# ProteusMRIgHIFU/BabelBrain

Measured on AMD Instinct MI355X. Metric: Mvoxel-steps/sec, 512^3 skull FDTD per device (achieved HBM GB/s in roofline), higher is better.
Workload: dtype f32

## Files before the change

babelbrain_amd/csrc/bfd_api.hip:

```cpp
#include "bfd_internal.h"

#include <math.h>
#include <stdio.h>
#include <string.h>

#include <algorithm>
#include <array>
#include <thread>
#include <hipcub/hipcub.hpp>

static thread_local std::string g_err;
void bfd_set_error(const std::string &s) { g_err = s; }

namespace {

struct HostTables {
    std::vector<float> t;
    float c1, k2;
    double cmax;
};

void fit_sls(double rho, double c, double alpha, double q, double omega, bool exact, double &MR, double &tau)
{
    if (c <= 0.0) { MR = 0.0; tau = 0.0; return; }
// ... 469 lines not shown
        BFD_FAIL(-2, "bfd_create: h, dt, freq must be > 0 and 0 < reflectionLimit < 1");
    int ndev = 0;
    if (hipGetDeviceCount(&ndev) != hipSuccess || ndev <= 0)
        BFD_FAIL(-3, "bfd_create: no HIP device available (this engine has no CPU fallback)");
    if (cfg->device < 0 || cfg->device >= ndev) BFD_FAIL(-3, "bfd_create: device ordinal out of range");
    BFD_HIP(hipSetDevice(cfg->device));

    bfd_sim *s = new bfd_sim();
    s->cfg = *cfg;
    s->step = 0; s->devBytes = 0; s->haveMaterials = s->haveMap = false; s->tilesReady = false;
    s->nSrcVox = 0; s->srcLin = s->srcRow = nullptr; s->srcW[0] = s->srcW[1] = s->srcW[2] = nullptr; s->pulseT = nullptr;
    s->nSources = s->lengthSource = 0;
    s->pulseHost = nullptr; s->tileSteps = s->nTiles = 0;
    s->srcK = 0; s->srcWeights = s->srcSignals = nullptr;
    for (int b = 0; b < 2; b++) { s->tileDev[b] = s->tilePinned[b] = nullptr; s->tileLoaded[b] = s->tilePacked[b] = -1; s->evTile[b] = nullptr; s->evTileUsed[b] = false; for (int q = 0; q < 2; q++) { s->evRead[b][q] = nullptr; s->evReadUsed[b][q] = false; } }
    s->sensEnt = nullptr; s->sensEntValid = false; s->sensIsBox = false; memset(s->sensBox, 0, sizeof s->sensBox);
    s->actBase = nullptr; s->actBytes = 0; s->actReady = false;
    s->nSensors = 0; s->sensLin = nullptr; s->sensOut = nullptr; s->dftAcc = nullptr; s->dftPk = nullptr; s->dftBin = 0;
    s->acc = s->pk = nullptr; s->timing = s->perKernel = false;
    s->pairEnv = true; s->pendingAcc = s->pairDone = false; s->pairedLaunches = 0;
    if (const char *ev = getenv("BFD_PAIR_ACC")) s->pairEnv = atoi(ev) != 0;
    s->advEnv = true; s->midStep = false; s->tiles.advVz = false;
    if (const char *ev = getenv("BFD_ADV_VZ")) s->advEnv = atoi(ev) != 0;
    s->tables = nullptr; s->profiles = nullptr; s->cmax = 0;
    memset(s->algBytes, 0, sizeof s->algBytes); s->tiles.ktimer = nullptr;
    if (hipStreamCreateWithFlags(&s->stream, hipStreamNonBlocking) != hipSuccess) { delete s; BFD_FAIL(-10, "hipStreamCreate failed"); }
    s->ownStream = true;
    if (hipEventCreate(&s->evBegin) != hipSuccess) { hipStreamDestroy(s->stream); delete s; BFD_FAIL(-10, "hipEventCreate failed"); }
    if (hipEventCreate(&s->evEnd) != hipSuccess) { hipEventDestroy(s->evBegin); hipStreamDestroy(s->stream); delete s; BFD_FAIL(-10, "hipEventCreate failed"); }

    bfd_dev &d = s->d;
    memset(&d, 0, sizeof d);
    d.N1 = cfg->N1; d.N2 = cfg->N2; d.N3 = cfg->N3; d.k0 = cfg->k0; d.nk = cfg->nk;
    d.ND = cfg->NDelta; d.P = P; d.plane = cfg->N1 * cfg->N2;
    s->nloc = (size_t)d.plane * d.nk;
    s->nalloc = (size_t)d.plane * (d.nk + 4);
    bfd_placement_cache_evict_other_sizes(cfg->device, s->nalloc * sizeof(float));

    int rc = 0;
    float **fp[15] = {&d.Vx, &d.Vy, &d.Vz, &d.Sxx, &d.Syy, &d.Szz, &d.Sxy, &d.Sxz, &d.Syz,
                      &d.Rxx, &d.Ryy, &d.Rzz, &d.Rxy, &d.Rxz, &d.Ryz};
    for (int a = 0; a < 15 && !rc; a++) {
        rc = dev_alloc(s, &s->stateBase[a], s->nalloc);
        if (!rc) *fp[a] = s->stateBase[a] + 2 * (size_t)d.plane;
    }
    if (!rc) rc = dev_alloc(s, &s->matBase, s->nalloc);
// ... 626 lines not shown
    const bool pairAcc = pair_engine(s, quiet_runs_wanted(s), T.nFluid);
    for (size_t r = 0; r < all.size(); r++) {
        const int4 &run = all[r];
        const int bx = run.x % tx, by = run.x / tx, kb = run.y & 0xFFFF, ke = run.y >> 16, f = run.z;
        const int xa = bx * 64, xb = std::min(xa + 64, N1), ya = by * 8, yb = std::min(ya + 8, N2);
        const double cells = (double)(xb - xa) * (yb - ya) * (ke - kb);
        const double inner = overlap(xa, xb, ND, N1 - ND) * overlap(ya, yb, ND, N2 - ND) * overlap(k0g + kb, k0g + ke, ND, N3 - ND);
        const bool fusedRun = r >= (size_t)(T.nFluid + T.nSolid);
        if (fusedRun) {
            const double fc = 64.0 * bfd_fused_rows() * (ke - kb);
            const double b = 32.0 + ((f & 2) ? 8.0 : 0.0) + ((f & 4) ? 0.0 : 2.0);
            B[0][BFD_K_FUSED] += b * fc; B[1][BFD_K_FUSED] += b * fc + 8.0 * fc;
        } else if (r < (size_t)T.nFluid) {
            const bool lossy = f & 2, uni = f & 4, single = (f & 16) != 0;
            double bs = 12.0 + 8.0 + (lossy ? 8.0 : 0.0) + (uni ? 0.0 : 2.0);
            if (!single) bs += 8.0 + (lossy ? 8.0 : 0.0);
            const double bv = 4.0 + 24.0 + (uni ? 0.0 : 2.0);
            for (int a = 0; a < 2; a++) { B[a][BFD_K_STRESS_FLUID] += bs * cells; B[a][BFD_K_VELOCITY_FLUID] += bv * cells; }
            if (pairAcc) B[1][BFD_K_STRESS_FLUID] += 4.0 * inner; else B[1][BFD_K_VELOCITY_FLUID] += 8.0 * inner;
            if (f & BFD_RUN_ADV_VZ) {
                const double advCells = (double)(xb - xa) * (yb - ya) * std::max(0, ke - kb - 3);
                for (int a = 0; a < 2; a++) { B[a][BFD_K_STRESS_FLUID] += 4.0 * advCells; B[a][BFD_K_VELOCITY_FLUID] -= 8.0 * advCells; }
            }
        } else if (s->cfg.kernelVariant == 2) {
            for (int a = 0; a < 2; a++) { B[a][BFD_K_STRESS_SOLID] += 110.0 * cells; B[a][BFD_K_VELOCITY_SOLID] += 50.0 * cells + (a ? 8.0 * inner : 0.0); }
        } else {
            for (int a = 0; a < 2; a++) B[a][BFD_K_VELOCITY_SOLID] += (a ? 8.0 * inner : 0.0);
        }
    }
    if (T.nSolid && s->cfg.kernelVariant != 2) {
        const double nF0 = (double)cnt[0], nF1 = (double)cnt[1], nS = (double)cnt[2] + (double)cnt[3], nE = (double)cnt[4], nR = (double)cnt[5];
        const double all = nF0 + nF1 + nS + nR;
        const double bs = 15.0 * all + 8.0 * nF0 + 16.0 * nF1 + 48.0 * nS + 48.0 * nR;
        const double bv = 31.0 * all + 8.0 * (nS + nR) + 4.0 * nE;
        const double bsf = 14.0 * all + 8.0 * nF0 + 16.0 * nF1 + 16.0 * nS + 8.0 * nR;
        for (int a = 0; a < 2; a++) { if (s->d.cssRow) B[a][BFD_K_STRESS_FLUID] += bsf; else B[a][BFD_K_STRESS_SOLID] += bs; B[a][BFD_K_VELOCITY_SOLID] += bv; }
    }
    if (s->tiles.nShear) {
        DevTemp<unsigned long long> dc; unsigned long long hc[2] = {0, 0};
        BFD_HIP(dc.alloc(2));
        hipMemsetAsync(dc, 0, sizeof hc, s->stream);
        hipLaunchKernelGGL(count_active_edges, dim3(grid_for(s->tiles.nShear)), dim3(256), 0, s->stream, s->tiles.shearCoef, s->tiles.shearCodes, s->tiles.nShear, dc.p);
        hipMemcpyAsync(hc, dc, sizeof hc, hipMemcpyDeviceToHost, s->stream);
        const hipError_t e = hipStreamSynchronize(s->stream);
        if (e != hipSuccess) BFD_FAIL(-10, std::string("shear edge count: ") + hipGetErrorString(e));
        s->tiles.nShearExplicit = (long)hc[1];
// ... 21 lines not shown
    dev_release(s, &s->tiles.cssRow); dev_release(s, &s->tiles.css); s->tiles.cssCap = 0; s->tiles.cssHosted = false;
    dev_release(s, &s->tiles.runsAll); s->tiles.nAll = s->tiles.nAllB = 0;
    dev_release(s, &s->tiles.runs); dev_release(s, &s->tiles.xmap); dev_release(s, &s->tiles.shearCells); dev_release(s, &s->tiles.shearCoef); dev_release(s, &s->tiles.shearR);
    dev_release(s, &s->tiles.shearCodes); dev_release(s, &s->tiles.shearTab);
    const TileGrid G = choose_tile_grid(s);
    std::vector<int> flags(G.n, 1), mats(G.n, 0);
    if (s->cfg.kernelVariant != 2) { const int rc = fetch_tile_classes(s, G.n, flags, mats); if (rc) return rc; }
    bfd_tiles &T = s->tiles;
    T.nMat = s->cfg.nMat;
    T.nFluid = T.nFluidB = T.nSolid = T.nSolidB = T.nSolidBP = T.nSolidIP = T.nFused = T.nLossless = T.nLossy = T.nSolidSub = T.nUni = T.nPml = T.nLean = T.nFusedSub = 0;
    s->d.tilesX = G.tx; s->d.tilesY = G.ty;
    if (s->cfg.kernelVariant != 2) for (int id = 0; id < G.n; id++) if (!(flags[id] & 1)) flags[id] |= 16;
    std::vector<int4> lists[5];
    std::vector<int4> listsAll[2];
    std::vector<char> taken((size_t)G.n, 0);
    form_fused_runs(s, G, flags, mats, taken, lists[4]);
    form_two_kernel_runs(s, G, flags, mats, taken, lists, listsAll);
    T.nFluidB = (int)lists[0].size(); T.nFluid = T.nFluidB + (int)lists[1].size();
    T.nSolidB = (int)lists[2].size(); T.nSolid = T.nSolidB + (int)lists[3].size();
    T.nFused = (int)lists[4].size();
    T.advVz = false;
    if (adv_vz_engine(s, T.nSolid))
        for (int a = 0; a < 2; a++)
            for (int4 &run : lists[a])
                if (!(run.z & (1 | 8)) && (run.y >> 16) - (run.y & 0xFFFF) >= 4) { run.z |= BFD_RUN_ADV_VZ; T.advVz = true; }
    std::vector<int4> all;
    for (int a = 0; a < 5; a++) all.insert(all.end(), lists[a].begin(), lists[a].end());
    int rc = dev_alloc(s, &s->tiles.runs, all.size(), false);
    if (rc) return rc;
    BFD_HIP(hipMemcpy(s->tiles.runs, all.data(), all.size() * sizeof(int4), hipMemcpyHostToDevice));
    rc = build_balance_maps(s, all);
    if (rc) return rc;
    s->tiles.nShearExplicit = 0;
    s->tiles.nShear = s->tiles.shearLowEnd = s->tiles.shearHighBeg = 0;
    if (T.nSolid && s->cfg.kernelVariant != 2) {
        int count = 0; bool compact = false; std::vector<unsigned> hostCells;
        rc = build_shear_list(s, G, &count, &compact, hostCells);
        if (!rc && compact) rc = setup_compact_state(s, G, count, listsAll);
        if (!rc && carryCompact) rc = carry_compact_in(s, count, oldCells, oldN, oldComp);
        if (!rc && compact && s->step > 0 && !carryCompact) {
            float *comp[10] = {s->d.cSxx, s->d.cSyy, s->d.cSxy, s->d.cSxz, s->d.cSyz, s->d.cRxx, s->d.cRyy, s->d.cRxy, s->d.cRxz, s->d.cRyz};
            for (int a = 0; a < 10; a++) BFD_HIP(hipMemsetAsync(comp[a], 0, (size_t)count * sizeof(float), s->stream));
            BFD_HIP(hipStreamSynchronize(s->stream));
        }
        if (rc) return rc;
        s->tiles.shearLowEnd = std::lower_bound(hostCells.begin(), hostCells.end(), (unsigned)G.lowPlanes * (unsigned)s->d.plane) - hostCells.begin();
        s->tiles.shearHighBeg = std::lower_bound(hostCells.begin(), hostCells.end(), (unsigned)G.hiStart * (unsigned)s->d.plane) - hostCells.begin();
    } else if (carryCompact) {
// ... 480 lines not shown
```

babelbrain_amd/csrc/bfd_internal.h:

```cpp
#pragma once
#include <hip/hip_runtime.h>
#include <stdint.h>
#include <algorithm>
#include <future>
#include <string>
#include <vector>
#include "../../include/babelfdtd.h"

#define BFD_REFLECTOR_BIT 0x8000u
#define BFD_MAT_MASK 0x7FFFu
#define BFD_CLS_FLUID 1u
#define BFD_CLS_NOMEM 2u
#define BFD_CLS_EXY 4u
#define BFD_CLS_EXZ 8u
#define BFD_CLS_EYZ 16u
#define BFD_CLS_REFL 32u

#ifndef BFD_CA
#define BFD_CA 1.125f
#define BFD_CB (1.0f / 24.0f)
#endif
#ifndef BFD_STAB
#define BFD_STAB (6.0 / 7.0)
#endif
// ... 24 lines not shown
    int actLo, actHi;
};
#define BFD_CSS_NONE 0xFFFFFFFFu
static __device__ __forceinline__ bool css_listed(unsigned c) { return (c & (BFD_CLS_FLUID | BFD_CLS_REFL)) == 0u; }
static __device__ __forceinline__ unsigned css_rank(bool listed)
{
    const unsigned long long b = __ballot(listed);
    return __builtin_amdgcn_mbcnt_hi((unsigned)(b >> 32), __builtin_amdgcn_mbcnt_lo((unsigned)b, 0u));
}
static __device__ __forceinline__ long css_index(const bfd_dev &d, long c)
{
    if (!css_listed(d.cls[c])) return -1;
    const int kl = (int)(c / d.plane);
    const int r = (int)(c - (long)kl * d.plane);
    const int j = r / d.N1, i = r - j * d.N1;
    const unsigned rb = d.cssRow[((long)(kl + 2) * d.N2 + j) * d.cssStride + (i >> 6)];
    if (rb == BFD_CSS_NONE) return -1;
    unsigned n = 0;
    for (long q = c - (i & 63); q < c; q++) n += css_listed(d.cls[q]) ? 1u : 0u;
    return (long)rb + n;
}

#define BFD_RUN_ADV_VZ 512
enum { BFD_K_STRESS_FLUID = 0, BFD_K_STRESS_SOLID = 1, BFD_K_STRESS_SHEAR = 2, BFD_K_VELOCITY_FLUID = 3, BFD_K_VELOCITY_SOLID = 4,
       BFD_K_FUSED = 5, BFD_K_COUNT = 6 };
struct bfd_sim;
void bfd_kmark(bfd_sim *sim, int cls, int end, hipStream_t st);

enum { BFD_XM_SF = 0, BFD_XM_VF = 3, BFD_XM_SS = 6, BFD_XM_VS = 9, BFD_XM_VSP_LO = 12, BFD_XM_VSP_HI = 13, BFD_XM_FUSED = 14, BFD_XMAP_COUNT = 15 };
struct bfd_tiles { bfd_sim *ktimer; int nMat; int4 *runs;
                   unsigned *shearCells; float *shearCoef; long nShear, shearLowEnd, shearHighBeg;
                   unsigned *shearCodes; float *shearTab; long nShearExplicit;
                   int4 *runsAll; int nAll, nAllB;
                   unsigned *cssRow; float *css; long cssCap; bool cssHosted;
                   float *shearR;
                   int nFluid, nFluidB, nSolid, nSolidB, nSolidBP , nSolidIP , nFused ;
                   int nLossless, nLossy, nSolidSub, nUni, nPml, nLean, nFusedSub;
                   bool advVz;
                   int *xmap; int xmapH[BFD_XMAP_COUNT][10]; };

struct bfd_sim {
    bfd_config cfg;
    bfd_dev d;
    hipStream_t stream;
    bool ownStream;
    int step;
// ... 11 lines not shown
    int64_t devBytes;
    bool haveMaterials, haveMap;
    bfd_tiles tiles; bool tilesReady;
    bool pingpong;
    float *ppBase[5];
    int zchunk;
    double cmax;
    int64_t nSrcVox, srcLowEnd, srcHighBeg;
    uint32_t *srcLin, *srcRow; float *srcW[3]; float *pulseT; int nSources, lengthSource;
    const double *pulseHost; int tileSteps, nTiles;
    float *tileDev[2], *tilePinned[2]; int tileLoaded[2], tilePacked[2];
    hipEvent_t evTile[2]; bool evTileUsed[2];
    hipEvent_t evRead[2][2]; bool evReadUsed[2][2];
    std::future<void> packJob[2];
    int srcK; float *srcWeights, *srcSignals;
    unsigned char *actBase; size_t actBytes; bool actReady;
    bool sensIsBox; int sensBox[5];
    int *sensEnt; bool sensEntValid;
    int64_t nSensors; uint32_t *sensLin; float *sensOut; int nTs; int nSelS; int selS[BFD_MAP_COUNT];
    double *dftAcc; float *dftPk; int dftBin;
    int nSelR; int selR[BFD_MAP_COUNT]; float *acc, *pk;
    int accStart;
    bool pairEnv, pendingAcc, pairDone; int64_t pairedLaunches;
    bool advEnv, midStep;
    bool timing, perKernel;
    hipEvent_t evBegin, evEnd;
    std::vector<hipEvent_t> evStress, evVelocity;
    std::vector<hipEvent_t> evK[BFD_K_COUNT];
    double algBytes[2][BFD_K_COUNT];
    std::vector<hipEvent_t> evPool;
    int *stepDev;
    hipGraphExec_t stepGraph;
    hipStream_t captureStream;
    int graphState;
    bool stepDevValid;
};
#define BFD_GRAPH_STEPS 8

void bfd_set_error(const std::string &s);
#define BFD_HIP(call)                                                                              \
    do {                                                                                           \
        hipError_t e_ = (call);                                                                    \
        if (e_ != hipSuccess) {                                                                    \
            bfd_set_error(std::string(#call) + ": " + hipGetErrorString(e_));                      \
            return -10;                                                                            \
        }                                                                                          \
    } while (0)
// ... 85 lines not shown
```

babelbrain_amd/csrc/bfd_kernels_v2.hip:

```cpp
#include "bfd_internal.h"
#include "bfd_device.h"
#include <algorithm>
#include <type_traits>

namespace {

constexpr int TX = BFD_TILE_X;
constexpr int TY = BFD_TILE_Y;
constexpr int LW = TX + 4;
constexpr int LH = TY + 4;
constexpr int NTHREADS = TX * TY;
constexpr int YT = 4 * TX;
constexpr int XT = 4 * TY;
constexpr int ZCHUNK = 32;
constexpr int SUBZ = BFD_SUBZ;
constexpr int STRESS_WAVES_PER_SIMD = 4;
constexpr int FLUID_WAVES_PER_SIMD = 8;
constexpr int VELOCITY_WAVES_PER_SIMD = 4;
constexpr int VELOCITY_FLUID_WAVES_PER_SIMD = FLUID_WAVES_PER_SIMD;

struct HaloTask {
    int lofs;
    int gofs;
    int arr;
// ... 396 lines not shown
__device__ __forceinline__ bool run_all_quiet(const bfd_dev &d, int bx, int by, int kbeg, int kend)
{
    const int q0 = kbeg / SUBZ, q1 = (kend - 1) / SUBZ;
    const int nq = q1 - q0 + 3;
    if (9 * nq > 64) return false;
    if (kbeg < d.actLo || kend > d.actHi) return false;
    const int l = threadIdx.x;
    const int dq = l / 9, r = l - 9 * dq, dy = r / 3, dx = r - 3 * dy;
    const unsigned idx = (unsigned)(((q0 + dq) * d.actY + (by + dy)) * d.actX + (bx + dx));
    const unsigned f = (l < 9 * nq) ? (unsigned)d.act[idx] : 0u;
    return __syncthreads_or(f != 0u) == 0;
}
__device__ __forceinline__ void run_mark_active(const bfd_dev &d, int bx, int by, int kbeg, int kend, unsigned nzbits)
{
    if (__ballot((nzbits & 0x7fffffffu) != 0u) == 0ull) return;
    if (threadIdx.x == 0)
        for (int q = kbeg / SUBZ; q <= (kend - 1) / SUBZ; q++) d.act[((q + 1) * d.actY + by + 1) * d.actX + bx + 1] = 1;
}
__device__ __forceinline__ unsigned fbits(float v) { return __float_as_uint(v); }

template <bool LOSSY, bool COLLAPSED, bool UNI, bool PML, bool SOLID = false, bool QUIET = false, bool PAIR = false>
__device__ __forceinline__ void stress_fluid_body(const bfd_dev &d, int bx, int by, int kbeg, int kend, int tm,
                                                  float (*sV)[2][LH * LW], float *__restrict__ accP = nullptr, float *__restrict__ pkP = nullptr,
                                                  bool advVz = false)
{
    constexpr bool ADVZ = !PML && !SOLID && !QUIET;
    static_assert(!PAIR || (!SOLID && !QUIET), "paired accumulation: plain fluid flavours only");
    unsigned nzb = 0u;
    const int N1 = d.N1, N2 = d.N2;
    const int tx = threadIdx.x, ty = threadIdx.y, tid = ty * TX + tx;
    const int i0 = bx * TX, j0 = by * TY;
    const int i = i0 + tx, j = j0 + ty;
    const bool valid = (i < N1) && (j < N2);
    const long pl = d.plane;
    const int P = d.P;
    const int own = (ty + 2) * LW + tx + 2;
    const unsigned cij = valid ? (unsigned)(j * N1 + i) : 0u;

    HaloTask t; t.lofs = -1; t.ok = false; t.arr = 0; t.gofs = 0;
    if (tid < YT) ytask(tid, 1, i0, j0, N1, N2, t);
    else if (tid < YT + XT) xtask(tid - YT, 0, i0, j0, N1, N2, t);
    const bool has = t.lofs >= 0;
    const float *ph = __builtin_amdgcn_readfirstlane(t.arr) == 0 ? d.Vx : d.Vy;
    const unsigned hofs = t.ok ? (unsigned)t.gofs * 4u : 0u;
    float *lh = &sV[0][t.arr][has ? t.lofs : 0];

    const float c1 = d.c1;
    float APu = 0.f, BPu = 0.f;
    if (UNI) { APu = d.AP[tm]; BPu = d.BP[tm]; }

    const bool zi = PML && valid && (i < P || i >= N1 - P);
    const bool zj = PML && valid && (j < P || j >= N2 - P);
    float ax = 0, bxc = 0, ay = 0, byc = 0, px = 0, py = 0, pz = 0;
    unsigned qx = 0, qy = 0;
    const unsigned dqx = (unsigned)(N2 * 2 * P), dqy = (unsigned)(2 * P * N1);
    if (PML) {
        if (zi) { ax = d.axI[i]; bxc = d.bxI[i]; qx = (unsigned)((kbeg * N2 + j) * (2 * P) + (i < P ? i : i - (N1 - 2 * P))); px = F4(d.psi[0], (unsigned)(qx) * 4u); }
        if (zj) { ay = d.ayI[j]; byc = d.byI[j]; qy = (unsigned)((kbeg * (2 * P) + (j < P ? j : j - (N2 - 2 * P))) * N1 + i); py = F4(d.psi[1], (unsigned)(qy) * 4u); }
        const int kg = d.k0 + kbeg;
        if (valid && (kg < P || kg >= d.N3 - P)) pz = F4(d.psi[2], (unsigned)((long)(kg < P ? kg : kg - (d.N3 - 2 * P)) * pl + cij) * 4u);
    }

    const bool inner = PAIR && valid && i >= d.ND && i < N1 - d.ND && j >= d.ND && j < N2 - d.ND;
    const bool accA = PAIR && accP != nullptr, accK = PAIR && pkP != nullptr;
    float vx0 = 0, vy0 = 0, vzm2 = 0, vzm1 = 0, vz0 = 0, vzp1 = 0, szz = 0, rzz = 0, av = 0;
    unsigned mraw = 0;
    if (valid) {
        const float *bVz = d.Vz + kbeg * pl;
        if (accA) av = LD4((accP + kbeg * pl), cij * 4u);
        vx0 = F4((d.Vx + kbeg * pl), cij * 4u); vy0 = F4((d.Vy + kbeg * pl), cij * 4u);
        vzm2 = LD4((bVz - 2 * pl), cij * 4u); vzm1 = LD4((bVz - pl), cij * 4u); vz0 = LD4(bVz, cij * 4u); vzp1 = LD4((bVz + pl), cij * 4u);
        szz = LD4((d.Szz + kbeg * pl), cij * 4u);
        if (LOSSY) rzz = LD4((d.Rzz + kbeg * pl), cij * 4u);
        if (!UNI) mraw = U2((d.mat + kbeg * pl), cij * 2u);
    }
    float hv = t.ok ? F4(ph + kbeg * pl, hofs) : 0.0f;
    float sq1 = 0, sq2 = 0, sq3 = 0, ruv = 0;
    unsigned mq1 = 0, mq2 = 0;
    if (ADVZ && UNI) ruv = d.invRho[tm];

    for (int kl = kbeg; kl < kend; kl++) {
        const int b = kl & 1;
        const long ko = (long)kl * pl;
        const int k = d.k0 + kl;
        sV[b][0][own] = vx0; sV[b][1][own] = vy0;
        if (has) lh[b * (2 * LH * LW)] = hv;
        float AP = APu, BP = BPu, AS2 = 0.f, BS2 = 0.f;
        if (!UNI && valid) { const int m = mraw & BFD_MAT_MASK; AP = d.AP[m]; if (LOSSY) BP = d.BP[m]; if (SOLID) { AS2 = d.AS2[m]; BS2 = d.BS2[m]; } }
        __syncthreads();

        float nvx = 0, nvy = 0, nvz = 0, nh = 0, nszz = 0, nrzz = 0, npx = 0, npy = 0, npz = 0, nav = 0, nsq = 0;
        unsigned nmraw = 0;
        if (kl + 1 < kend) {
            if (valid) {
                nvx = F4((d.Vx + ko + pl), cij * 4u); nvy = F4((d.Vy + ko + pl), cij * 4u); nvz = LD4((d.Vz + ko + 2 * pl), cij * 4u);
                nszz = LD4((d.Szz + ko + pl), cij * 4u);
                if (accA) nav = LD4((accP + ko + pl), cij * 4u);
                if (LOSSY) nrzz = LD4((d.Rzz + ko + pl), cij * 4u);
                if (!UNI) nmraw = U2((d.mat + ko + pl), cij * 2u);
            }
            if (t.ok) nh = F4(ph + ko + pl, hofs);
            if (PML) {
                if (zi) npx = F4(d.psi[0], (unsigned)(qx + dqx) * 4u);
                if (zj) npy = F4(d.psi[1], (unsigned)(qy + dqy) * 4u);
                const int kn = k + 1;
                if (valid && (kn < P || kn >= d.N3 - P)) npz = F4(d.psi[2], (unsigned)((long)(kn < P ? kn : kn - (d.N3 - 2 * P)) * pl + cij) * 4u);
            }
        }
        if (valid) {
            const float *sx = &sV[b][0][own], *sy = &sV[b][1][own];
            float dxVx = dminus4(sx[-2], sx[-1], vx0, sx[1]);
            float dyVy = dminus4(sy[-2 * LW], sy[-LW], vy0, sy[LW]);
            float dzVz = dminus4(vzm2, vzm1, vz0, vzp1);
            float val = 0.f, rn = 0.f;
            if (UNI || !(mraw & BFD_REFLECTOR_BIT)) {
                if (PML) {
                    if (zi) { const float pn = bxc * px + ax * dxVx; F4(d.psi[0], (unsigned)(qx) * 4u) = pn; dxVx = dxVx + pn; }
                    if (zj) { const float pn = byc * py + ay * dyVy; F4(d.psi[1], (unsigned)(qy) * 4u) = pn; dyVy = dyVy + pn; }
                    if (k < P || k >= d.N3 - P) {
                        const float pn = d.bzI[k] * pz + d.azI[k] * dzVz;
                        F4(d.psi[2], (unsigned)((long)(k < P ? k : k - (d.N3 - 2 * P)) * pl + cij) * 4u) = pn;
                        dzVz = dzVz + pn;
                    }
                }
                const float sXY = dxVx + dyVy;
                const float div = sXY + dzVz;
                if (SOLID) {
                    rn = c1 * rzz - (BP * div - BS2 * sXY);
                    val = szz + ((AP * div - AS2 * sXY) + 0.5f * (rzz + rn));
                } else if (LOSSY) {
                    rn = c1 * rzz - BP * div;
// ... 5 lines not shown
            ST4((d.SzzW + ko), cij * 4u, val);
            if (PAIR) {
                if (inner && k >= d.ND && k < d.N3 - d.ND) {
                    const float so = (szz + szz) + szz, sn = (val + val) + val;
                    const float po = -so * (1.0f / 3.0f), pn = -sn * (1.0f / 3.0f);
                    if (accA) ST4((accP + ko), cij * 4u, (av + po * po) + pn * pn);
                    if (accK) {
                        const float m0 = F4((pkP + ko), cij * 4u), ao = fabsf(po), an = fabsf(pn);
                        float m = m0;
                        if (ao > m) m = ao;
                        if (an > m) m = an;
                        if (m > m0) F4((pkP + ko), cij * 4u) = m;
                    }
                }
            }
            if (QUIET) nzb |= fbits(val) | fbits(rn);
            if (!COLLAPSED) { F4((d.Sxx + ko), cij * 4u) = val; F4((d.Syy + ko), cij * 4u) = val; }
            if (LOSSY) {
                ST4((d.RzzW + ko), cij * 4u, rn);
                if (!COLLAPSED) { F4((d.Rxx + ko), cij * 4u) = rn; F4((d.Ryy + ko), cij * 4u) = rn; }
            }
            if (ADVZ) {
                nsq = val;
                if (advVz && kl >= kbeg + 3) {
                    float r0 = ruv, r1 = ruv;
                    if (!UNI) { r0 = d.invRho[mq2 & BFD_MAT_MASK]; r1 = d.invRho[mq1 & BFD_MAT_MASK]; }
                    const float dz = dplus4(sq3, sq2, sq1, val);
                    float w = vzm2 + (0.5f * (r0 + r1)) * dz;
                    if (!UNI && (mq2 & BFD_REFLECTOR_BIT)) w = 0.f;
                    ST4((d.VzW + ko - 2 * pl), cij * 4u, w);
                }
            }
        }
        if (ADVZ) { sq3 = sq2; sq2 = sq1; sq1 = nsq; mq2 = mq1; mq1 = mraw; }
        vx0 = nvx; vy0 = nvy;
        vzm2 = vzm1; vzm1 = vz0; vz0 = vzp1; vzp1 = nvz;
        hv = nh; szz = nszz; rzz = nrzz; mraw = nmraw; av = nav;
        px = npx; py = npy; pz = npz; qx += dqx; qy += dqy;
    }
    if (QUIET) run_mark_active(d, bx, by, kbeg, kend, nzb);
}

template <bool ACC, bool UNI, bool PML, bool QUIET = false>
__device__ __forceinline__ void velocity_fluid_body(const bfd_dev &d, int bx, int by, int kbeg, int kend, int tm,
                                                    float (*sS)[LH * LW], float *__restrict__ accP, float *__restrict__ pkP, bool advVz = false)
{
    const bool adv = !PML && !QUIET && advVz;
    const int N1 = d.N1, N2 = d.N2;
    const int tx = threadIdx.x, ty = threadIdx.y, tid = ty * TX + tx;
    const int i0 = bx * TX, j0 = by * TY;
    const int i = i0 + tx, j = j0 + ty;
    const bool valid = (i < N1) && (j < N2);
    const long pl = d.plane;
    const int P = d.P;
    const int own = (ty + 2) * LW + tx + 2;
    const unsigned cij = valid ? (unsigned)(j * N1 + i) : 0u;
    const unsigned cx = valid ? (unsigned)(j * N1 + min(i + 1, N1 - 1)) : 0u;
    const unsigned cy = valid ? (unsigned)(min(j + 1, N2 - 1) * N1 + i) : 0u;

    HaloTask t; t.lofs = -1; t.ok = false; t.arr = 0; t.gofs = 0;
    if (tid < YT) ytask(tid, 0, i0, j0, N1, N2, t);
    else if (tid < YT + XT) xtask(tid - YT, 0, i0, j0, N1, N2, t);
    const bool has = t.lofs >= 0;
    const float *ph = d.Szz;
    const unsigned hofs = t.ok ? (unsigned)t.gofs * 4u : 0u;
    float *lh = &sS[0][has ? t.lofs : 0];

    const bool inner = valid && i >= d.ND && i < N1 - d.ND && j >= d.ND && j < N2 - d.ND;
    const bool accA = ACC && accP != nullptr, accK = ACC && pkP != nullptr;
    unsigned nzb = 0u;
    float ru = 0.f;
    if (UNI) ru = d.invRho[tm];

    const bool zi = PML && valid && (i < P || i >= N1 - P);
    const bool zj = PML && valid && (j < P || j >= N2 - P);
    float ax = 0, bxc = 0, ay = 0, byc = 0, px = 0, py = 0, pz = 0;
    unsigned qx = 0, qy = 0;
    const unsigned dqx = (unsigned)(N2 * 2 * P), dqy = (unsigned)(2 * P * N1);
    if (PML) {
        if (zi) { ax = d.axH[i]; bxc = d.bxH[i]; qx = (unsigned)((kbeg * N2 + j) * (2 * P) + (i < P ? i : i - (N1 - 2 * P))); px = F4(d.psi[9], (unsigned)(qx) * 4u); }
        if (zj) { ay = d.ayH[j]; byc = d.byH[j]; qy = (unsigned)((kbeg * (2 * P) + (j < P ? j : j - (N2 - 2 * P))) * N1 + i); py = F4(d.psi[13], (unsigned)(qy) * 4u); }
        const int kg = d.k0 + kbeg;
        if (valid && (kg < P || kg >= d.N3 - P)) pz = F4(d.psi[17], (unsigned)((long)(kg < P ? kg : kg - (d.N3 - 2 * P)) * pl + cij) * 4u);
    }

    float sm1 = 0, s0 = 0, sp1 = 0, sp2 = 0, vx = 0, vy = 0, vz = 0, av = 0, r0 = ru;
    unsigned mraw = 0, mraw1 = 0, mx = 0, my = 0;
    if (valid) {
        const float *bS = d.Szz + kbeg * pl;
        sm1 = F4((bS - pl), cij * 4u); s0 = F4(bS, cij * 4u); sp1 = F4((bS + pl), cij * 4u); sp2 = F4((bS + 2 * pl), cij * 4u);
        vx = LD4((d.Vx + kbeg * pl), cij * 4u); vy = LD4((d.Vy + kbeg * pl), cij * 4u); vz = LD4((d.Vz + kbeg * pl), cij * 4u);
        if (accA) av = LD4((accP + kbeg * pl), cij * 4u);
        if (!UNI) {
            const uint16_t *bM = d.mat + kbeg * pl;
            mraw = U2(bM, cij * 2u); mraw1 = U2((bM + pl), cij * 2u); mx = U2(bM, cx * 2u); my = U2(bM, cy * 2u);
            r0 = d.invRho[mraw & BFD_MAT_MASK];
        }
    }
    float hv = t.ok ? F4(ph + kbeg * pl, hofs) : 0.0f;

    for (int kl = kbeg; kl < kend; kl++) {
        const int b = kl & 1;
        const long ko = (long)kl * pl;
        const int k = d.k0 + kl;
        sS[b][own] = s0;
        if (has) lh[b * (LH * LW)] = hv;
        float r1 = ru, rx = ru, ry = ru;
        if (!UNI && valid) {
            r1 = d.invRho[mraw1 & BFD_MAT_MASK];
            rx = d.invRho[mx & BFD_MAT_MASK];
            ry = d.invRho[my & BFD_MAT_MASK];
        }
        __syncthreads();

        float ns = 0, nh = 0, nvx = 0, nvy = 0, nvz = 0, nav = 0, npx = 0, npy = 0, npz = 0;
        unsigned nm2 = 0, nmx = 0, nmy = 0;
        if (!UNI && valid) nm2 = U2((d.mat + ko + 2 * pl), cij * 2u);
        if (kl + 1 < kend) {
            if (valid) {
                ns = F4((d.Szz + ko + 3 * pl), cij * 4u);
                nvx = LD4((d.Vx + ko + pl), cij * 4u); nvy = LD4((d.Vy + ko + pl), cij * 4u);
                if (!(adv && kl + 1 < kend - 2)) nvz = LD4((d.Vz + ko + pl), cij * 4u);
                if (!UNI) { nmx = U2((d.mat + ko + pl), cx * 2u); nmy = U2((d.mat + ko + pl), cy * 2u); }
                if (accA) nav = LD4((accP + ko + pl), cij * 4u);
            }
            if (t.ok) nh = F4(ph + ko + pl, hofs);
            if (PML) {
                if (zi) npx = F4(d.psi[9], (unsigned)(qx + dqx) * 4u);
                if (zj) npy = F4(d.psi[13], (unsigned)(qy + dqy) * 4u);
                const int kn = k + 1;
                if (valid && (kn < P || kn >= d.N3 - P)) npz = F4(d.psi[17], (unsigned)((long)(kn < P ? kn : kn - (d.N3 - 2 * P)) * pl + cij) * 4u);
            }
        }
        const bool ownVz = !(adv && kl > kbeg && kl < kend - 2);
        if (valid) {
            if (ACC) {
                if (inner && k >= d.ND && k < d.N3 - d.ND) {
                    const float s = (s0 + s0) + s0;
                    const float p = -s * (1.0f / 3.0f);
                    if (accA) ST4((accP + ko), cij * 4u, av + p * p);
                    if (accK) { const float ap = fabsf(p); if (ap > F4((pkP + ko), cij * 4u)) F4((pkP + ko), cij * 4u) = ap; }
                }
            }
            if (!UNI && (mraw & BFD_REFLECTOR_BIT)) {
                F4((d.VxW + ko), cij * 4u) = 0.f; F4((d.VyW + ko), cij * 4u) = 0.f;
                if (ownVz) F4((d.VzW + ko), cij * 4u) = 0.f;
            } else {
                const float *p = &sS[b][own];
                float dx = dplus4(p[-1], s0, p[1], p[2]);
                float dy = dplus4(p[-LW], s0, p[LW], p[2 * LW]);
                float dz = dplus4(sm1, s0, sp1, sp2);
                if (PML) {
                    if (zi) { const float pn = bxc * px + ax * dx; F4(d.psi[9], (unsigned)(qx) * 4u) = pn; dx = dx + pn; }
                    if (zj) { const float pn = byc * py + ay * dy; F4(d.psi[13], (unsigned)(qy) * 4u) = pn; dy = dy + pn; }
                    if (k < P || k >= d.N3 - P) {
                        const float pn = d.bzH[k] * pz + d.azH[k] * dz;
                        F4(d.psi[17], (unsigned)((long)(k < P ? k : k - (d.N3 - 2 * P)) * pl + cij) * 4u) = pn;
                        dz = dz + pn;
                    }
                }
                if (!QUIET) {
                    ST4((d.VxW + ko), cij * 4u, vx + (0.5f * (r0 + rx)) * dx);
                    ST4((d.VyW + ko), cij * 4u, vy + (0.5f * (r0 + ry)) * dy);
                    if (ownVz) ST4((d.VzW + ko), cij * 4u, vz + (0.5f * (r0 + r1)) * dz);
                } else {
                    { const float w = vx + (0.5f * (r0 + rx)) * dx; ST4((d.VxW + ko), cij * 4u, w); nzb |= fbits(w); }
                    { const float w = vy + (0.5f * (r0 + ry)) * dy; ST4((d.VyW + ko), cij * 4u, w); nzb |= fbits(w); }
                    { const float w = vz + (0.5f * (r0 + r1)) * dz; ST4((d.VzW + ko), cij * 4u, w); nzb |= fbits(w); }
                }
            }
        }
        sm1 = s0; s0 = sp1; sp1 = sp2; sp2 = ns;
        hv = nh; vx = nvx; vy = nvy; vz = nvz; av = nav;
        r0 = r1; mraw = mraw1; mraw1 = nm2; mx = nmx; my = nmy;
        px = npx; py = npy; pz = npz; qx += dqx; qy += dqy;
    }
    if (QUIET) run_mark_active(d, bx, by, kbeg, kend, nzb);
}

template <bool PML>
__device__ __forceinline__ void stress_solid_body(const bfd_dev &d, const int4 &run, int tilesX, float (*sV)[2][LH * LW])
{
    const int N1 = d.N1, N2 = d.N2;
    const int bx = run.x % tilesX, by = run.x / tilesX, kbeg = run.y & 0xFFFF, kend = run.y >> 16;
    const int tx = threadIdx.x, ty = threadIdx.y, tid = ty * TX + tx;
    const int i0 = bx * TX, j0 = by * TY;
// ... 738 lines not shown
    }
    for (int q = 0; q < 6; q++) coef[6 * t + q] = o[q];
    if (codes) {
        auto code = [&](float A, int ma, int mb, int mc) { return A == 0.f ? 0u : ((m == ma && m == mb && m == mc && m < 254) ? (unsigned)(1 + m) : 255u); };
        codes[t] = code(o[0], mx, my, mxy) | (code(o[2], mx, mz, mxz) << 8) | (code(o[4], my, mz, myz) << 16) | (m < 255 ? (unsigned)(1 + m) << 24 : 0u);
    }
}
__global__ void shear_material_table(bfd_dev d, float *__restrict__ tab, int nMat)
{
    const int m = blockIdx.x * blockDim.x + threadIdx.x;
    if (m >= nMat) return;
    const float iv0 = d.invMu[m], t0 = d.tauS[m], k2 = d.k2;
    float A = 0.f, B = 0.f;
    if (iv0 > 0.f) {
        const float muH = 4.0f / ((iv0 + iv0) + (iv0 + iv0));
        const float tau = 0.25f * ((t0 + t0) + (t0 + t0));
        A = muH * (1.0f + tau); B = (muH * tau) * k2;
    }
    tab[8 * m] = A; tab[8 * m + 1] = B; tab[8 * m + 2] = 0.f; tab[8 * m + 3] = 0.f;
    tab[8 * m + 4] = d.AP[m]; tab[8 * m + 5] = d.BP[m]; tab[8 * m + 6] = d.AS2[m]; tab[8 * m + 7] = d.BS2[m];
}

template <bool COLLAPSED, bool QUIET = false, bool PAIR = false>
__device__ __forceinline__ void stress_fluid_switch(const bfd_dev &d, const int4 &run, int tilesX, float (*sV)[2][LH * LW],
                                                    float *__restrict__ accP = nullptr, float *__restrict__ pkP = nullptr)
{
    const int bx = run.x % tilesX, by = run.x / tilesX, kbeg = run.y & 0xFFFF, kend = run.y >> 16, tm = run.w;
    const bool adv = (run.z & BFD_RUN_ADV_VZ) != 0;
    if (QUIET && run_all_quiet(d, bx, by, kbeg, kend)) return;
    if (run.z & 1) {
        if (run.z & 8) stress_fluid_body<true, true, false, true, true, QUIET>(d, bx, by, kbeg, kend, tm, sV);
        else stress_fluid_body<true, true, false, false, true, QUIET>(d, bx, by, kbeg, kend, tm, sV);
        return;
    }
    switch ((run.z >> 1) & 7) {
    case 0: stress_fluid_body<false, COLLAPSED, false, false, false, QUIET, PAIR>(d, bx, by, kbeg, kend, tm, sV, accP, pkP, adv); break;
    case 1: stress_fluid_body<true, COLLAPSED, false, false, false, QUIET, PAIR>(d, bx, by, kbeg, kend, tm, sV, accP, pkP, adv); break;
    case 2: stress_fluid_body<false, COLLAPSED, true, false, false, QUIET, PAIR>(d, bx, by, kbeg, kend, tm, sV, accP, pkP, adv); break;
    case 3: stress_fluid_body<true, COLLAPSED, true, false, false, QUIET, PAIR>(d, bx, by, kbeg, kend, tm, sV, accP, pkP, adv); break;
    case 4: stress_fluid_body<false, COLLAPSED, false, true, false, QUIET, PAIR>(d, bx, by, kbeg, kend, tm, sV, accP, pkP); break;
    case 5: stress_fluid_body<true, COLLAPSED, false, true, false, QUIET, PAIR>(d, bx, by, kbeg, kend, tm, sV, accP, pkP); break;
    case 6: stress_fluid_body<false, COLLAPSED, true, true, false, QUIET, PAIR>(d, bx, by, kbeg, kend, tm, sV, accP, pkP); break;
    default: stress_fluid_body<true, COLLAPSED, true, true, false, QUIET, PAIR>(d, bx, by, kbeg, kend, tm, sV, accP, pkP); break;
    }
}

template <bool COLLAPSED, bool QUIET = false, bool PAIR = false>
__global__ __launch_bounds__(NTHREADS, FLUID_WAVES_PER_SIMD) void stress_fluid(bfd_dev d, int tilesX, int nblocks, const int *__restrict__ xmap,
                                                                               const int4 *__restrict__ runs,
                                                                               float *__restrict__ accP, float *__restrict__ pkP)
{
    __shared__ float sV[2][2][LH * LW];
    const int ri = run_index(nblocks, xmap);
    if (ri < 0) return;
    const int4 run = runs[ri];
    if (COLLAPSED || (run.z & 16)) stress_fluid_switch<true, QUIET, PAIR>(d, run, tilesX, sV, accP, pkP);
    else stress_fluid_switch<false, QUIET, PAIR>(d, run, tilesX, sV, accP, pkP);
}

__global__ __launch_bounds__(NTHREADS) void flush_paired_pressure(bfd_dev d, int tilesX, int nruns, const int4 *__restrict__ runs,
                                                                  float *__restrict__ accP, float *__restrict__ pkP)
{
    if ((int)blockIdx.x >= nruns) return;
    const int4 run = runs[blockIdx.x];
    const int bx = run.x % tilesX, by = run.x / tilesX, kbeg = run.y & 0xFFFF, kend = run.y >> 16;
    const int i = bx * TX + (int)threadIdx.x, j = by * TY + (int)threadIdx.y;
    if (!(i >= d.ND && i < d.N1 - d.ND && j >= d.ND && j < d.N2 - d.ND)) return;
    const long cij = (long)j * d.N1 + i;
    for (int kl = kbeg; kl < kend; kl++) {
        const int k = d.k0 + kl;
        if (k < d.ND || k >= d.N3 - d.ND) continue;
        const long c = (long)kl * d.plane + cij;
        const float s0 = d.Szz[c];
        const float s = (s0 + s0) + s0;
        const float p = -s * (1.0f / 3.0f);
        if (accP) accP[c] = accP[c] + p * p;
        if (pkP) { const float ap = fabsf(p); if (ap > pkP[c]) pkP[c] = ap; }
    }
}

template <bool ACC, bool QUIET = false>
__global__ __launch_bounds__(NTHREADS, VELOCITY_FLUID_WAVES_PER_SIMD) void velocity_fluid(bfd_dev d, int tilesX, int nblocks, const int *__restrict__ xmap,
                                                                                 const int4 *__restrict__ runs,
                                                                                 float *__restrict__ accP, float *__restrict__ pkP)
{
    __shared__ float sS[2][LH * LW];
    const int ri = run_index(nblocks, xmap);
    if (ri < 0) return;
    const int4 run = runs[ri];
    const int bx = run.x % tilesX, by = run.x / tilesX, kbeg = run.y & 0xFFFF, kend = run.y >> 16, tm = run.w;
    const bool adv = (run.z & BFD_RUN_ADV_VZ) != 0;
    if (QUIET && run_all_quiet(d, bx, by, kbeg, kend)) return;
    switch ((run.z >> 2) & 3) {
    case 0: velocity_fluid_body<ACC, false, false, QUIET>(d, bx, by, kbeg, kend, tm, sS, accP, pkP, adv); break;
    case 1: velocity_fluid_body<ACC, true, false, QUIET>(d, bx, by, kbeg, kend, tm, sS, accP, pkP, adv); break;
    case 2: velocity_fluid_body<ACC, false, true, QUIET>(d, bx, by, kbeg, kend, tm, sS, accP, pkP); break;
    default: velocity_fluid_body<ACC, true, true, QUIET>(d, bx, by, kbeg, kend, tm, sS, accP, pkP); break;
    }
}

__global__ void classify_tiles(bfd_dev d, int tilesX, int tilesY, int *__restrict__ flags, int *__restrict__ tileMat)
{
    const int tile = blockIdx.x;
    const int bx = tile % tilesX, by = (tile / tilesX) % tilesY, bz = tile / (tilesX * tilesY);
    const int i0 = bx * TX - 2, j0 = by * TY - 2, k0 = bz * SUBZ - 2;
    const int nzOwn = min(SUBZ, d.nk - bz * SUBZ);
    const int nx = TX + 4, ny = TY + 4, nz = nzOwn + 4;
    const unsigned first = d.mat[(long)(bz * SUBZ) * d.plane + (long)min(by * TY, d.N2 - 1) * d.N1 + min(bx * TX, d.N1 - 1)];
    int solid = 0, lossy = 0, lossyG = 0, refl = 0, mixed = (first & BFD_REFLECTOR_BIT) ? 1 : 0;
    for (int v = threadIdx.x; v < nx * ny * nz; v += blockDim.x) {
        const int li = v % nx, lj = (v / nx) % ny, lk = v / (nx * ny);
        const int i = i0 + li, j = j0 + lj, kl = k0 + lk;
        if (i < 0 || i >= d.N1 || j < 0 || j >= d.N2) continue;
        const unsigned raw = d.mat[(long)kl * d.plane + (long)j * d.N1 + i];
        const int m = raw & BFD_MAT_MASK;
        if (raw != first) mixed = 1;
        if (raw & BFD_REFLECTOR_BIT) refl = 1;
        if (d.invMu[m] > 0.f) solid = 1;
// ... 265 lines not shown
```

Measured before the change: 97490.

## Advance Vy in the fluid stress kernel for interior tile rows

Extends the existing 'advance Vz in the stress kernel' trick to Vy. For interior rows of full tiles, the fluid stress kernel now stages the fresh pressure and inverse density in a new shared buffer. It then computes and stores the updated Vy one plane behind, and the velocity kernel skips loading and storing Vy for those rows. Halo task assignments are trimmed to match. This removes a read and a write of Vy per voxel from the velocity pass, at the cost of extra shared memory, an extra barrier and more register pressure in the stress kernel.

```diff
diff --git a/babelbrain_amd/csrc/bfd_api.hip b/babelbrain_amd/csrc/bfd_api.hip
--- a/babelbrain_amd/csrc/bfd_api.hip
+++ b/babelbrain_amd/csrc/bfd_api.hip
@@ -515,6 +515,8 @@
     if (const char *ev = getenv("BFD_PAIR_ACC")) s->pairEnv = atoi(ev) != 0;
     s->advEnv = true; s->midStep = false; s->tiles.advVz = false;
     if (const char *ev = getenv("BFD_ADV_VZ")) s->advEnv = atoi(ev) != 0;
+    s->advVyEnv = true;
+    if (const char *ev = getenv("BFD_ADV_VY")) s->advVyEnv = atoi(ev) != 0;
     s->tables = nullptr; s->profiles = nullptr; s->cmax = 0;
     memset(s->algBytes, 0, sizeof s->algBytes); s->tiles.ktimer = nullptr;
     if (hipStreamCreateWithFlags(&s->stream, hipStreamNonBlocking) != hipSuccess) { delete s; BFD_FAIL(-10, "hipStreamCreate failed"); }
@@ -1187,6 +1189,10 @@
                 const double advCells = (double)(xb - xa) * (yb - ya) * std::max(0, ke - kb - 3);
                 for (int a = 0; a < 2; a++) { B[a][BFD_K_STRESS_FLUID] += 4.0 * advCells; B[a][BFD_K_VELOCITY_FLUID] -= 8.0 * advCells; }
             }
+            if (f & BFD_RUN_ADV_VY) {
+                const double advCells = 64.0 * 5.0 * (ke - kb);
+                for (int a = 0; a < 2; a++) { B[a][BFD_K_STRESS_FLUID] += 4.0 * advCells; B[a][BFD_K_VELOCITY_FLUID] -= 8.0 * advCells; }
+            }
         } else if (s->cfg.kernelVariant == 2) {
             for (int a = 0; a < 2; a++) { B[a][BFD_K_STRESS_SOLID] += 110.0 * cells; B[a][BFD_K_VELOCITY_SOLID] += 50.0 * cells + (a ? 8.0 * inner : 0.0); }
         } else {
@@ -1254,8 +1260,12 @@
     T.advVz = false;
     if (adv_vz_engine(s, T.nSolid))
         for (int a = 0; a < 2; a++)
-            for (int4 &run : lists[a])
-                if (!(run.z & (1 | 8)) && (run.y >> 16) - (run.y & 0xFFFF) >= 4) { run.z |= BFD_RUN_ADV_VZ; T.advVz = true; }
+            for (int4 &run : lists[a]) {
+                if (run.z & (1 | 8)) continue;
+                if ((run.y >> 16) - (run.y & 0xFFFF) >= 4) { run.z |= BFD_RUN_ADV_VZ; T.advVz = true; }
+                const int bx = run.x % G.tx, by = run.x / G.tx;
+                if (s->advVyEnv && s->d.VyW == s->d.Vy && (bx + 1) * 64 <= s->d.N1 && (by + 1) * 8 <= s->d.N2) { run.z |= BFD_RUN_ADV_VY; T.advVz = true; }
+            }
     std::vector<int4> all;
     for (int a = 0; a < 5; a++) all.insert(all.end(), lists[a].begin(), lists[a].end());
     int rc = dev_alloc(s, &s->tiles.runs, all.size(), false);
diff --git a/babelbrain_amd/csrc/bfd_internal.h b/babelbrain_amd/csrc/bfd_internal.h
--- a/babelbrain_amd/csrc/bfd_internal.h
+++ b/babelbrain_amd/csrc/bfd_internal.h
@@ -70,6 +70,7 @@
 }
 
 #define BFD_RUN_ADV_VZ 512
+#define BFD_RUN_ADV_VY 1024
 enum { BFD_K_STRESS_FLUID = 0, BFD_K_STRESS_SOLID = 1, BFD_K_STRESS_SHEAR = 2, BFD_K_VELOCITY_FLUID = 3, BFD_K_VELOCITY_SOLID = 4,
        BFD_K_FUSED = 5, BFD_K_COUNT = 6 };
 struct bfd_sim;
@@ -127,7 +128,7 @@
     int nSelR; int selR[BFD_MAP_COUNT]; float *acc, *pk;
     int accStart;
     bool pairEnv, pendingAcc, pairDone; int64_t pairedLaunches;
-    bool advEnv, midStep;
+    bool advEnv, advVyEnv, midStep;
     bool timing, perKernel;
     hipEvent_t evBegin, evEnd;
     std::vector<hipEvent_t> evStress, evVelocity;
diff --git a/babelbrain_amd/csrc/bfd_kernels_v2.hip b/babelbrain_amd/csrc/bfd_kernels_v2.hip
--- a/babelbrain_amd/csrc/bfd_kernels_v2.hip
+++ b/babelbrain_amd/csrc/bfd_kernels_v2.hip
@@ -442,7 +442,7 @@
 template <bool LOSSY, bool COLLAPSED, bool UNI, bool PML, bool SOLID = false, bool QUIET = false, bool PAIR = false>
 __device__ __forceinline__ void stress_fluid_body(const bfd_dev &d, int bx, int by, int kbeg, int kend, int tm,
                                                   float (*sV)[2][LH * LW], float *__restrict__ accP = nullptr, float *__restrict__ pkP = nullptr,
-                                                  bool advVz = false)
+                                                  bool advVz = false, bool advVy = false, float (*sQ)[2][NTHREADS] = nullptr)
 {
     constexpr bool ADVZ = !PML && !SOLID && !QUIET;
     static_assert(!PAIR || (!SOLID && !QUIET), "paired accumulation: plain fluid flavours only");
@@ -458,8 +458,8 @@
     const unsigned cij = valid ? (unsigned)(j * N1 + i) : 0u;
 
     HaloTask t; t.lofs = -1; t.ok = false; t.arr = 0; t.gofs = 0;
-    if (tid < YT) ytask(tid, 1, i0, j0, N1, N2, t);
-    else if (tid < YT + XT) xtask(tid - YT, 0, i0, j0, N1, N2, t);
+    if (tid < 3 * TX) ytask(tid, 1, i0, j0, N1, N2, t);
+    else if (tid >= YT && tid < YT + XT && ((tid - YT) & 3) != 3) xtask(tid - YT, 0, i0, j0, N1, N2, t);
     const bool has = t.lofs >= 0;
     const float *ph = __builtin_amdgcn_readfirstlane(t.arr) == 0 ? d.Vx : d.Vy;
     const unsigned hofs = t.ok ? (unsigned)t.gofs * 4u : 0u;
@@ -498,6 +498,17 @@
     float sq1 = 0, sq2 = 0, sq3 = 0, ruv = 0;
     unsigned mq1 = 0, mq2 = 0;
     if (ADVZ && UNI) ruv = d.invRho[tm];
+    const bool rowAdvVy = ADVZ && advVy && ty >= 1 && ty <= TY - 3;
+    auto advance_vy = [&](int kl) {
+        const int pb = (kl - 1) & 1;
+        const float *q = &sQ[pb][0][tid];
+        const float dy = dplus4(q[-TX], sq1, q[TX], q[2 * TX]);
+        float r0 = ruv, ry = ruv;
+        if (!UNI) { r0 = sQ[pb][1][tid]; ry = sQ[pb][1][tid + TX]; }
+        float w = sV[pb][1][own] + (0.5f * (r0 + ry)) * dy;
+        if (!UNI && (mq1 & BFD_REFLECTOR_BIT)) w = 0.f;
+        ST4((d.VyW + (long)(kl - 1) * pl), cij * 4u, w);
+    };
 
     for (int kl = kbeg; kl < kend; kl++) {
         const int b = kl & 1;
@@ -505,8 +516,11 @@
         const int k = d.k0 + kl;
         sV[b][0][own] = vx0; sV[b][1][own] = vy0;
         if (has) lh[b * (2 * LH * LW)] = hv;
-        float AP = APu, BP = BPu, AS2 = 0.f, BS2 = 0.f;
-        if (!UNI && valid) { const int m = mraw & BFD_MAT_MASK; AP = d.AP[m]; if (LOSSY) BP = d.BP[m]; if (SOLID) { AS2 = d.AS2[m]; BS2 = d.BS2[m]; } }
+        float AP = APu, BP = BPu, AS2 = 0.f, BS2 = 0.f, rq = 0.f;
+        if (!UNI && valid) {
+            const int m = mraw & BFD_MAT_MASK; AP = d.AP[m]; if (LOSSY) BP = d.BP[m]; if (SOLID) { AS2 = d.AS2[m]; BS2 = d.BS2[m]; }
+            if (ADVZ && advVy) rq = d.invRho[m];
+        }
         __syncthreads();
 
         float nvx = 0, nvy = 0, nvz = 0, nh = 0, nszz = 0, nrzz = 0, npx = 0, npy = 0, npz = 0, nav = 0, nsq = 0;
@@ -527,6 +541,7 @@
                 if (valid && (kn < P || kn >= d.N3 - P)) npz = F4(d.psi[2], (unsigned)((long)(kn < P ? kn : kn - (d.N3 - 2 * P)) * pl + cij) * 4u);
             }
         }
+        if (rowAdvVy && kl > kbeg) advance_vy(kl);
         if (valid) {
             const float *sx = &sV[b][0][own], *sy = &sV[b][1][own];
             float dxVx = dminus4(sx[-2], sx[-1], vx0, sx[1]);
@@ -578,6 +593,7 @@
             }
             if (ADVZ) {
                 nsq = val;
+                if (advVy) { sQ[b][0][tid] = val; if (!UNI) sQ[b][1][tid] = rq; }
                 if (advVz && kl >= kbeg + 3) {
                     float r0 = ruv, r1 = ruv;
                     if (!UNI) { r0 = d.invRho[mq2 & BFD_MAT_MASK]; r1 = d.invRho[mq1 & BFD_MAT_MASK]; }
@@ -594,12 +610,17 @@
         hv = nh; szz = nszz; rzz = nrzz; mraw = nmraw; av = nav;
         px = npx; py = npy; pz = npz; qx += dqx; qy += dqy;
     }
+    if (ADVZ && advVy) {
+        __syncthreads();
+        if (rowAdvVy) advance_vy(kend);
+    }
     if (QUIET) run_mark_active(d, bx, by, kbeg, kend, nzb);
 }
 
 template <bool ACC, bool UNI, bool PML, bool QUIET = false>
 __device__ __forceinline__ void velocity_fluid_body(const bfd_dev &d, int bx, int by, int kbeg, int kend, int tm,
-                                                    float (*sS)[LH * LW], float *__restrict__ accP, float *__restrict__ pkP, bool advVz = false)
+                                                    float (*sS)[LH * LW], float *__restrict__ accP, float *__restrict__ pkP, bool advVz = false,
+                                                    bool advVy = false)
 {
     const bool adv = !PML && !QUIET && advVz;
     const int N1 = d.N1, N2 = d.N2;
@@ -615,10 +636,11 @@
     const unsigned cy = valid ? (unsigned)(min(j + 1, N2 - 1) * N1 + i) : 0u;
 
     HaloTask t; t.lofs = -1; t.ok = false; t.arr = 0; t.gofs = 0;
-    if (tid < YT) ytask(tid, 0, i0, j0, N1, N2, t);
-    else if (tid < YT + XT) xtask(tid - YT, 0, i0, j0, N1, N2, t);
+    if (tid >= TX && tid < YT) ytask(tid, 0, i0, j0, N1, N2, t);
+    else if (tid >= YT && tid < YT + XT && ((tid - YT) & 3) != 0) xtask(tid - YT, 0, i0, j0, N1, N2, t);
     const bool has = t.lofs >= 0;
     const float *ph = d.Szz;
+    const bool ownVy = !(!PML && !QUIET && advVy && ty >= 1 && ty <= TY - 3);
     const unsigned hofs = t.ok ? (unsigned)t.gofs * 4u : 0u;
     float *lh = &sS[0][has ? t.lofs : 0];
 
@@ -645,7 +667,7 @@
     if (valid) {
         const float *bS = d.Szz + kbeg * pl;
         sm1 = F4((bS - pl), cij * 4u); s0 = F4(bS, cij * 4u); sp1 = F4((bS + pl), cij * 4u); sp2 = F4((bS + 2 * pl), cij * 4u);
-        vx = LD4((d.Vx + kbeg * pl), cij * 4u); vy = LD4((d.Vy + kbeg * pl), cij * 4u); vz = LD4((d.Vz + kbeg * pl), cij * 4u);
+        vx = LD4((d.Vx + kbeg * pl), cij * 4u); if (ownVy) vy = LD4((d.Vy + kbeg * pl), cij * 4u); vz = LD4((d.Vz + kbeg * pl), cij * 4u);
         if (accA) av = LD4((accP + kbeg * pl), cij * 4u);
         if (!UNI) {
             const uint16_t *bM = d.mat + kbeg * pl;
@@ -675,7 +697,7 @@
         if (kl + 1 < kend) {
             if (valid) {
                 ns = F4((d.Szz + ko + 3 * pl), cij * 4u);
-                nvx = LD4((d.Vx + ko + pl), cij * 4u); nvy = LD4((d.Vy + ko + pl), cij * 4u);
+                nvx = LD4((d.Vx + ko + pl), cij * 4u); if (ownVy) nvy = LD4((d.Vy + ko + pl), cij * 4u);
                 if (!(adv && kl + 1 < kend - 2)) nvz = LD4((d.Vz + ko + pl), cij * 4u);
                 if (!UNI) { nmx = U2((d.mat + ko + pl), cx * 2u); nmy = U2((d.mat + ko + pl), cy * 2u); }
                 if (accA) nav = LD4((accP + ko + pl), cij * 4u);
@@ -699,7 +721,7 @@
                 }
             }
             if (!UNI && (mraw & BFD_REFLECTOR_BIT)) {
-                F4((d.VxW + ko), cij * 4u) = 0.f; F4((d.VyW + ko), cij * 4u) = 0.f;
+                F4((d.VxW + ko), cij * 4u) = 0.f; if (ownVy) F4((d.VyW + ko), cij * 4u) = 0.f;
                 if (ownVz) F4((d.VzW + ko), cij * 4u) = 0.f;
             } else {
                 const float *p = &sS[b][own];
@@ -717,7 +739,7 @@
                 }
                 if (!QUIET) {
                     ST4((d.VxW + ko), cij * 4u, vx + (0.5f * (r0 + rx)) * dx);
-                    ST4((d.VyW + ko), cij * 4u, vy + (0.5f * (r0 + ry)) * dy);
+                    if (ownVy) ST4((d.VyW + ko), cij * 4u, vy + (0.5f * (r0 + ry)) * dy);
                     if (ownVz) ST4((d.VzW + ko), cij * 4u, vz + (0.5f * (r0 + r1)) * dz);
                 } else {
                     { const float w = vx + (0.5f * (r0 + rx)) * dx; ST4((d.VxW + ko), cij * 4u, w); nzb |= fbits(w); }
@@ -1502,11 +1524,11 @@
 }
 
 template <bool COLLAPSED, bool QUIET = false, bool PAIR = false>
-__device__ __forceinline__ void stress_fluid_switch(const bfd_dev &d, const int4 &run, int tilesX, float (*sV)[2][LH * LW],
+__device__ __forceinline__ void stress_fluid_switch(const bfd_dev &d, const int4 &run, int tilesX, float (*sV)[2][LH * LW], float (*sQ)[2][NTHREADS],
                                                     float *__restrict__ accP = nullptr, float *__restrict__ pkP = nullptr)
 {
     const int bx = run.x % tilesX, by = run.x / tilesX, kbeg = run.y & 0xFFFF, kend = run.y >> 16, tm = run.w;
-    const bool adv = (run.z & BFD_RUN_ADV_VZ) != 0;
+    const bool adv = (run.z & BFD_RUN_ADV_VZ) != 0, advY = !QUIET && (run.z & BFD_RUN_ADV_VY) != 0;
     if (QUIET && run_all_quiet(d, bx, by, kbeg, kend)) return;
     if (run.z & 1) {
         if (run.z & 8) stress_fluid_body<true, true, false, true, true, QUIET>(d, bx, by, kbeg, kend, tm, sV);
@@ -1514,10 +1536,10 @@
         return;
     }
     switch ((run.z >> 1) & 7) {
-    case 0: stress_fluid_body<false, COLLAPSED, false, false, false, QUIET, PAIR>(d, bx, by, kbeg, kend, tm, sV, accP, pkP, adv); break;
-    case 1: stress_fluid_body<true, COLLAPSED, false, false, false, QUIET, PAIR>(d, bx, by, kbeg, kend, tm, sV, accP, pkP, adv); break;
-    case 2: stress_fluid_body<false, COLLAPSED, true, false, false, QUIET, PAIR>(d, bx, by, kbeg, kend, tm, sV, accP, pkP, adv); break;
-    case 3: stress_fluid_body<true, COLLAPSED, true, false, false, QUIET, PAIR>(d, bx, by, kbeg, kend, tm, sV, accP, pkP, adv); break;
+    case 0: stress_fluid_body<false, COLLAPSED, false, false, false, QUIET, PAIR>(d, bx, by, kbeg, kend, tm, sV, accP, pkP, adv, advY, sQ); break;
+    case 1: stress_fluid_body<true, COLLAPSED, false, false, false, QUIET, PAIR>(d, bx, by, kbeg, kend, tm, sV, accP, pkP, adv, advY, sQ); break;
+    case 2: stress_fluid_body<false, COLLAPSED, true, false, false, QUIET, PAIR>(d, bx, by, kbeg, kend, tm, sV, accP, pkP, adv, advY, sQ); break;
+    case 3: stress_fluid_body<true, COLLAPSED, true, false, false, QUIET, PAIR>(d, bx, by, kbeg, kend, tm, sV, accP, pkP, adv, advY, sQ); break;
     case 4: stress_fluid_body<false, COLLAPSED, false, true, false, QUIET, PAIR>(d, bx, by, kbeg, kend, tm, sV, accP, pkP); break;
     case 5: stress_fluid_body<true, COLLAPSED, false, true, false, QUIET, PAIR>(d, bx, by, kbeg, kend, tm, sV, accP, pkP); break;
     case 6: stress_fluid_body<false, COLLAPSED, true, true, false, QUIET, PAIR>(d, bx, by, kbeg, kend, tm, sV, accP, pkP); break;
@@ -1531,11 +1553,12 @@
                                                                                float *__restrict__ accP, float *__restrict__ pkP)
 {
     __shared__ float sV[2][2][LH * LW];
+    __shared__ float sQ[QUIET ? 1 : 2][2][QUIET ? 1 : NTHREADS];
     const int ri = run_index(nblocks, xmap);
     if (ri < 0) return;
     const int4 run = runs[ri];
-    if (COLLAPSED || (run.z & 16)) stress_fluid_switch<true, QUIET, PAIR>(d, run, tilesX, sV, accP, pkP);
-    else stress_fluid_switch<false, QUIET, PAIR>(d, run, tilesX, sV, accP, pkP);
+    if (COLLAPSED || (run.z & 16)) stress_fluid_switch<true, QUIET, PAIR>(d, run, tilesX, sV, (float (*)[2][NTHREADS])sQ, accP, pkP);
+    else stress_fluid_switch<false, QUIET, PAIR>(d, run, tilesX, sV, (float (*)[2][NTHREADS])sQ, accP, pkP);
 }
 
 __global__ __launch_bounds__(NTHREADS) void flush_paired_pressure(bfd_dev d, int tilesX, int nruns, const int4 *__restrict__ runs,
@@ -1569,11 +1592,11 @@
     if (ri < 0) return;
     const int4 run = runs[ri];
     const int bx = run.x % tilesX, by = run.x / tilesX, kbeg = run.y & 0xFFFF, kend = run.y >> 16, tm = run.w;
-    const bool adv = (run.z & BFD_RUN_ADV_VZ) != 0;
+    const bool adv = (run.z & BFD_RUN_ADV_VZ) != 0, advY = (run.z & BFD_RUN_ADV_VY) != 0;
     if (QUIET && run_all_quiet(d, bx, by, kbeg, kend)) return;
     switch ((run.z >> 2) & 3) {
-    case 0: velocity_fluid_body<ACC, false, false, QUIET>(d, bx, by, kbeg, kend, tm, sS, accP, pkP, adv); break;
-    case 1: velocity_fluid_body<ACC, true, false, QUIET>(d, bx, by, kbeg, kend, tm, sS, accP, pkP, adv); break;
+    case 0: velocity_fluid_body<ACC, false, false, QUIET>(d, bx, by, kbeg, kend, tm, sS, accP, pkP, adv, advY); break;
+    case 1: velocity_fluid_body<ACC, true, false, QUIET>(d, bx, by, kbeg, kend, tm, sS, accP, pkP, adv, advY); break;
     case 2: velocity_fluid_body<ACC, false, true, QUIET>(d, bx, by, kbeg, kend, tm, sS, accP, pkP); break;
     default: velocity_fluid_body<ACC, true, true, QUIET>(d, bx, by, kbeg, kend, tm, sS, accP, pkP); break;
     }
```

Measured after the change: 97220 (median of 2 runs). No clear change (-0.3%).
